# ucuapps/OpenGlue

Measured on AMD Instinct MI355X. Metric: image-pairs/sec (1024 kpts, 256-dim, 9 GNN layers), higher is better.
Workload: dtype f32; 1 GPU; BASELINE configs[1]: 1024x1024 kpts, 256-dim, 9 self+cross stages, 4 heads, 100 Sinkhorn iters, batch=32 pairs/GPU, random-init weights, seeded synthetic keypoints/descriptors; global_batch=32, pairs_per_gpu=32, parallelism=pairs sharded over 1 GPU(s), 1 RCCL gather

## Files before the change

openglue_amd/build.py:

```python
from __future__ import annotations

import argparse
import os
import shutil
import subprocess
import sys
from concurrent.futures import ThreadPoolExecutor

HERE = os.path.dirname(os.path.abspath(__file__))
CSRC = os.path.join(HERE, "csrc")
LIB_DIR = os.path.join(HERE, "lib")
LIB_PATH = os.path.join(LIB_DIR, "libopenglue_amd.so")
SOURCES = ["gemm_f32.hip", "gemm_f16x3.hip", "mlp_fused.hip", "attention.hip", "attention_train.hip", "linear_attention.hip", "sinkhorn.hip", "sinkhorn_resident.hip", "sinkhorn_train.hip", "batchnorm_train.hip", "matches.hip", "features.hip", "supervision.hip", "metrics.hip", "superpoint.hip", "optimizer.hip", "api.hip"]
ARCH = "gfx950"


def _hipcc() -> str:
    for cand in (os.environ.get("HIPCC"), shutil.which("hipcc"), "/opt/rocm/bin/hipcc"):
        if cand and os.path.exists(cand):
            return cand
    raise RuntimeError("hipcc not found (set HIPCC or install ROCm under /opt/rocm)")


_NO_PACKED_FP32 = ["-Xclang", "-target-feature", "-Xclang", "-packed-fp32-ops"]
PER_FILE_FLAGS = {"attention.hip": _NO_PACKED_FP32}
FLAGS = ["--offload-arch=" + ARCH, "-std=c++17", "-fPIC", "-O3", "-Wall", "-Wno-unused-function"]


def _stale(target: str, deps) -> bool:
    if not os.path.exists(target):
        return True
    t = os.path.getmtime(target)
    return any(os.path.getmtime(d) > t for d in deps)


def build(force: bool = False, debug: bool = False, verbose: bool = True) -> str:
    os.makedirs(LIB_DIR, exist_ok=True)
    hipcc = _hipcc()
    headers = [os.path.join(CSRC, "og_common.h"), os.path.join(os.path.dirname(HERE), "include", "openglue_amd.h")]
    flags = list(FLAGS)
    if debug:
        flags += ["-g", "-save-temps=obj"]
    objs, jobs = [], []
    for src in SOURCES:
        sp = os.path.join(CSRC, src)
        op = os.path.join(LIB_DIR, src.replace(".hip", ".o"))
        objs.append(op)
        if force or _stale(op, [sp, *headers, os.path.abspath(__file__)]):
            jobs.append([hipcc, *flags, *PER_FILE_FLAGS.get(src, []), "-c", sp, "-o", op])

    def run(cmd):
        if verbose:
            print(" ".join(cmd), flush=True)
        r = subprocess.run(cmd, capture_output=True, text=True)
        if r.returncode != 0:
            raise RuntimeError("hipcc failed:\n" + r.stdout + r.stderr)
        err = "\n".join(l for l in r.stderr.splitlines() if "is not a recognized feature for this target" not in l)
        if err.strip() and verbose:
            print(err, file=sys.stderr)

    with ThreadPoolExecutor(max_workers=max(1, min(len(jobs), os.cpu_count() or 1))) as ex:
        list(ex.map(run, jobs))
    if jobs or force or _stale(LIB_PATH, objs):
        run([hipcc, "--offload-arch=" + ARCH, "-shared", "-fPIC", "-o", LIB_PATH, *objs])
    return LIB_PATH


if __name__ == "__main__":
    ap = argparse.ArgumentParser()
    ap.add_argument("--force", action="store_true")
    ap.add_argument("--debug", action="store_true")
    a = ap.parse_args()
    print(build(force=a.force, debug=a.debug))
```

openglue_amd/csrc/api.hip:

```cpp
#include <math.h>
#include <cmath>
#include <stdlib.h>
#include <string.h>
#include <vector>
#include <dlfcn.h>
#include <stdio.h>

#include "og_common.h"

namespace {

constexpr double BN_EPS = 1e-5;

struct PackedLayout {
    int n_enc;
    int enc_k[OG_MAX_HIDDEN + 1];
    int enc_out[OG_MAX_HIDDEN + 1];
    int64_t enc_w[OG_MAX_HIDDEN + 1], enc_b[OG_MAX_HIDDEN + 1];
    int64_t enc_whl;
    int64_t layer0, layer_stride;
    int64_t o_wqkv, o_bqkv, o_w0, o_b0, o_w3, o_b3;
    int64_t o_wmlp;
    int64_t o_wqkvs;
    int64_t o_wqkvb;
// ... 363 lines not shown
            push = (int (*)(const char*))dlsym(h, "roctxRangePushA");
            pop = (int (*)())dlsym(h, "roctxRangePop");
            if (push && pop) return;
            push = nullptr; pop = nullptr;
        }
    }
};
struct Range {
    static const Roctx& rt() { static const Roctx r; return r; }
    bool on;
    explicit Range(const char* name) : on(rt().push != nullptr) { if (on) rt().push(name); }
    Range(const char* name, int idx) : on(rt().push != nullptr) {
        if (on) { char buf[48]; snprintf(buf, sizeof buf, "%s %d", name, idx); rt().push(buf); }
    }
    ~Range() { if (on) rt().pop(); }
    Range(const Range&) = delete;
};
struct Scope {
    Profiler* p; int i;
    Scope(Profiler* pp, int c) : p(pp), i(pp ? pp->begin(c) : -1) {}
    ~Scope() { if (p) p->end(i); }
};

int forward_impl(const og_shape* shape, const og_inputs* in, const void* packed_dev, void* workspace_dev,
                 const og_outputs* outp, void* stream, Profiler* prof, const RaggedDesc* rag = nullptr,
                 const EncoderRagged* er0 = nullptr, const EncoderRagged* er1 = nullptr, int tap = -1, float* tap_x = nullptr,
                 bool encoder_only = false) {
    static const og_outputs no_outputs{};
    if (encoder_only && !outp) outp = &no_outputs;
    if (!shape || !in || !packed_dev || !workspace_dev || !outp) return OG_E_INVALID;
    if (int e = check_shape(shape)) return e;
    og_clear_status();
    const og_shape& s = *shape;
    if (!in->keypoints0 || !in->keypoints1 || !in->descriptors0 || !in->descriptors1 || (!outp->scores && !encoder_only)) return OG_E_INVALID;
    if (s.side_info > 0 && (!in->side_info0 || !in->side_info1)) return OG_E_INVALID;
    if ((outp->matches0 == nullptr) != (outp->matching_scores0 == nullptr)) return OG_E_INVALID;
    if ((outp->matches1 == nullptr) != (outp->matching_scores1 == nullptr)) return OG_E_INVALID;
    if (outp->matches1 && !outp->matches0) return OG_E_INVALID;
    if (((uintptr_t)packed_dev & 15) || ((uintptr_t)workspace_dev & 15) || ((uintptr_t)in->descriptors0 & 15) ||
        ((uintptr_t)in->descriptors1 & 15))
        return OG_E_ALIGN;
    hipStream_t st = (hipStream_t)stream;
    const PackedLayout L = packed_layout(s);
    const WorkspaceLayout W = workspace_layout(s);
    const float* pk = (const float*)packed_dev;
    float* ws = (float*)workspace_dev;
    const int D = s.desc_dim, D2 = 2 * D, B = s.batch, m = s.m, n = s.n;
    const bool favor = s.flags & OG_FLAG_FAVOR_RELU;
    const int WQ = qk_width(s), QW = qkv_width(s);
    const int64_t T0 = rag ? rag->off0[B] : (int64_t)B * m, T1 = rag ? rag->off1[B] : (int64_t)B * n, T = T0 + T1;
    float* X32 = ws + W.x32; float* G = ws + W.g; float* Sb = ws + W.sbuf;
    const int D4 = 4 * D;
    _Float16* XO = (_Float16*)(ws + W.xo);
    _Float16* QKVh = (_Float16*)(ws + W.qkvh); _Float16* QKVl = (_Float16*)(ws + W.qkvl);
    _Float16* Hb = (_Float16*)(ws + W.h);
    int rc;

    auto gemm = [&](const float* A, int64_t lda, const float* Bm, int64_t ldb, float* C, int64_t ldc, int64_t M, int N, int K,
                    const float* bias, int relu, const float* res, int64_t ldr, _Float16* Chl, int64_t ldch) -> int {
        GemmArgs g{};
        g.A = A; g.lda = lda; g.strideA = 0; g.B = Bm; g.ldb = ldb; g.strideB = 0; g.C = C; g.ldc = ldc; g.strideC = 0;
        g.M = (int)M; g.N = N; g.K = K; g.batch = 1; g.bias = bias; g.relu = relu; g.res = res; g.ldr = ldr; g.strideR = 0;
        g.alpha = nullptr; g.scale = 1.f; g.Ct = nullptr; g.ldct = 0; g.strideCt = 0; g.ct_rows = 1;
        g.Ch = Chl; g.Cl = Chl ? Chl + 32 : nullptr; g.ldch = ldch; g.c_hl = 1;
        Scope sc(prof, OG_STAGE_GEMM);
        return og_launch_gemm(g, st);
    };
    auto gemmh = [&](const _Float16* A, const float* wbase, int64_t o_w, int64_t wrow0, int64_t M, int N, int K,
                     const float* bias, int relu, const _Float16* res_hl, float* C32, _Float16* Ch, _Float16* Cl, int64_t ldch,
                     int c_hl) -> int {
        GemmHArgs g{};
        g.scale_dev = wbase + L.o_scale + (o_w == L.o_wqkv ? 0 : o_w == L.o_w0 ? 1 : 2);
        g.A = A; g.lda = D4;
        g.B = (const _Float16*)(wbase + o_w) + wrow0 * 2 * K; g.ldb = 2 * K;
        g.M = (int)M; g.N = N; g.K = K; g.scale = (float)(1.0 / OG_W_SCALE); g.bias = bias; g.relu = relu; g.res = nullptr; g.ldr = D; g.res_hl = res_hl; g.ldrh = D4;
        g.C32 = C32; g.ldc = D; g.Ch = Ch; g.Cl = Cl; g.ldch = ldch; g.c_hl = c_hl;
        Scope sc(prof, OG_STAGE_GEMM_F16X3);
        return og_launch_gemm_f16x3(g, st);
    };

    Range r_forward("og_forward");
    {
        Range r_stage("encoder");
        float* EI = ws + W.ei;
        float* Ea = ws + W.ea;
        float* Eb = ws + W.eb;
        {
            Scope sc(prof, OG_STAGE_ENCODER_INPUT);
            if ((rc = og_launch_encoder_input(in->keypoints0, in->side_info0, T0, s.side_info, in->image0_wh[0], in->image0_wh[1], EI, st, er0))) return rc;
            if ((rc = og_launch_encoder_input(in->keypoints1, in->side_info1, T1, s.side_info, in->image1_wh[0], in->image1_wh[1], EI + T0 * 32, st, er1))) return rc;
        }
        const float* cur = EI; int64_t ldcur = 32;
        const bool tail_f16 = L.enc_whl >= 0;
        const int last = L.n_enc - 1;
        _Float16* Ehl = (_Float16*)G;
        for (int i = 0; i < L.n_enc; ++i) {
            const float* Wi = pk + L.enc_w[i]; const float* bi = pk + L.enc_b[i];
            if (i < last) {
                float* dst = (i & 1) ? Eb : Ea;
                const int act = (s.flags & OG_FLAG_SIREN_ENCODER) ? 2 : 1;
                const bool to_hl = tail_f16 && i == last - 1;
                if ((rc = gemm(cur, ldcur, Wi, L.enc_k[i], to_hl ? nullptr : dst, L.enc_maxw, T, L.enc_out[i], L.enc_k[i], bi, act, nullptr, 0,
                               to_hl ? Ehl : nullptr, to_hl ? 2 * L.enc_out[i] : 0))) return rc;
                cur = dst; ldcur = L.enc_maxw;
            } else {
                const bool nd = s.flags & OG_FLAG_NO_DESCRIPTORS;
                const float* res[2] = {nd ? nullptr : in->descriptors0, nd ? nullptr : in->descriptors1};
                const int64_t r0[2] = {0, T0}, R[2] = {T0, T1};
                for (int side = 0; side < 2; ++side) {
                    if (tail_f16) {
                        const int K = L.enc_k[i];
                        GemmHArgs g{};
                        g.A = Ehl + r0[side] * 2 * K; g.lda = 2 * K;
                        g.B = (const _Float16*)(pk + L.enc_whl); g.ldb = 2 * K;
                        g.M = (int)R[side]; g.N = D; g.K = K; g.scale = (float)(1.0 / OG_W_SCALE); g.scale_dev = pk + L.scales + 1; g.bias = bi; g.relu = 0;
                        g.res = res[side]; g.ldr = D; g.res_hl = nullptr; g.ldrh = 0;
                        g.C32 = nullptr; g.ldc = D; g.Ch = XO + r0[side] * D4; g.Cl = g.Ch + 32; g.ldch = D4; g.c_hl = 1;
                        Scope sc(prof, OG_STAGE_GEMM_F16X3);
                        if ((rc = og_launch_gemm_f16x3(g, st))) return rc;
                    } else {
                        if ((rc = gemm(cur + r0[side] * ldcur, ldcur, Wi, L.enc_k[i], X32 + r0[side] * D, D, R[side], D, L.enc_k[i], bi, 0, res[side], D,
                                       XO + r0[side] * D4, D4))) return rc;
                    }
                }
            }
        }
    }

    auto tap_here = [&](int idx) -> int {
        if (tap != idx || !tap_x) return 0;
        return og_launch_merge_f16_hl(XO, T, D, D4, tap_x, D, st);
    };
    if ((rc = tap_here(0))) return rc;
    if (encoder_only) return og_launch_status();

    const int dh = D / s.num_heads;
    if (hipMemsetAsync(ws + W.attn, 0, OG_ATTN_COUNTERS * sizeof(int), st) != hipSuccess) return OG_E_INVALID;
    auto attention = [&](int nz, int split, int64_t qb0, int64_t qs0, int nq0, int64_t kb0, int64_t ks0, int nk0,
                         int64_t qb1, int64_t qs1, int nq1, int64_t kb1, int64_t ks1, int nk1, int rag_mode) -> int {
        AttnArgs a{};
        a.rag = rag; a.rag_mode = rag_mode;
        a.qh = QKVh; a.ql = QKVl; a.ldq = QW; a.kh = QKVh + WQ; a.kl = QKVl + WQ; a.ldk = QW;
        a.vh = QKVh + 2 * WQ; a.vl = QKVl + 2 * WQ; a.ldv = QW;
        a.feat = favor ? WQ : 0;
        a.oh = XO + D2; a.ol = XO + D2 + 32; a.ldo = D4; a.o_hl = 1;
        a.nz = nz; a.num_heads = s.num_heads; a.dh = dh; a.split = split;
        a.counters = reinterpret_cast<int*>(ws + W.attn); a.partial = ws + W.attn + OG_ATTN_COUNTERS;
        a.q_base[0] = qb0; a.q_step[0] = qs0; a.nq[0] = nq0; a.kv_base[0] = kb0; a.kv_step[0] = ks0; a.nk[0] = nk0;
        a.q_base[1] = qb1; a.q_step[1] = qs1; a.nq[1] = nq1; a.kv_base[1] = kb1; a.kv_step[1] = ks1; a.nk[1] = nk1;
        Scope sc(prof, OG_STAGE_ATTENTION);
        if (favor) return og_launch_favor_attention(a, st);
        return (s.flags & OG_FLAG_LINEAR_ATTENTION) ? og_launch_linear_attention(a, st) : og_launch_attention(a, st);
    };
    auto proj_small_ok = [&](int64_t R) {
        static const int mode = [] { const char* e = getenv("OG_PROJ_SMALL"); return e ? atoi(e) : -1; }();
        return L.o_wqkvs >= 0 && !favor && (mode >= 0 ? mode != 0 : R <= 8192) && R < ((int64_t)1 << 30);
    };
    auto proj_small = [&](const float* lw, int64_t r0, int64_t R, int split_row, int a0, int a1, int b0, int b1) -> int {
        Scope sc(prof, OG_STAGE_GEMM_F16X3);
        return og_launch_proj_small(XO + r0 * D4, D4, (int)R, D, (const char*)(lw + L.o_wqkvs), lw + L.o_bqkv, lw + L.o_scale,
                                    QKVh + r0 * QW, QKVl + r0 * QW, QW, split_row, a0, a1, b0, b1, st);
    };
    auto proj_stream_ok = [&](int64_t R, bool full = false) {
        return L.o_wqkvb >= 0 && !favor && og_proj_stream_wanted((int)(R < ((int64_t)1 << 30) ? R : 0), D, full) && R < ((int64_t)1 << 30) && QW % 64 == 0 &&
               !(((uintptr_t)QKVh | (uintptr_t)QKVl) & 127);
    };
    auto proj_stream = [&](const float* lw, int64_t r0, int64_t R, int split_row, int a0, int a1, int b0, int b1) -> int {
        Scope sc(prof, OG_STAGE_GEMM_F16X3);
        return og_launch_proj_stream(XO + r0 * D4, D4, (int)R, D, (const char*)(lw + L.o_wqkvb), lw + L.o_bqkv, lw + L.o_scale,
                                     QKVh + r0 * QW, QKVl + r0 * QW, QW, split_row, a0 / 128, a1 / 128, b0 / 128, b1 / 128, st);
    };
    auto qkv_proj = [&](const float* lw, int64_t r0, int64_t R, int c0, int c1) -> int {
        if (proj_small_ok(R) && c0 % 32 == 0 && c1 % 32 == 0) return proj_small(lw, r0, R, 0, 0, 0, c0 / 32, c1 / 32);
        if (proj_stream_ok(R, c0 == 0 && c1 == QW) && c0 % 128 == 0 && c1 % 128 == 0 && ((r0 * QW * 2) % 128 == 0)) return proj_stream(lw, r0, R, 0, 0, 0, c0, c1);
        const int cut = favor ? 2 * WQ : c1;
        const int ca[2] = {c0, c0 < cut && cut < c1 ? cut : c1}, cb[2] = {ca[1], c1};
        for (int part = 0; part < 2; ++part) {
            const int a0 = part ? cb[0] : ca[0], a1 = part ? cb[1] : ca[1];
            if (a1 <= a0) continue;
// ... 213 lines not shown
```

openglue_amd/csrc/og_common.h:

```cpp
#pragma once
#include <hip/hip_runtime.h>
#include <stdint.h>
#include "../../include/openglue_amd.h"

typedef float f32x4 __attribute__((ext_vector_type(4)));
typedef float f32x16 __attribute__((ext_vector_type(16)));
typedef _Float16 f16x4 __attribute__((ext_vector_type(4)));
typedef _Float16 f16x8 __attribute__((ext_vector_type(8)));

#define OG_WAVE 64
#define OG_NEG_INF (-__builtin_huge_valf())

__device__ __forceinline__ int mfma32_row(int r, int lane) { return (r & 3) + 8 * (r >> 2) + 4 * (lane >> 5); }

__device__ __forceinline__ float wave_max(float v) {
#pragma unroll
    for (int o = 32; o > 0; o >>= 1) v = fmaxf(v, __shfl_xor(v, o, 64));
    return v;
}
__device__ __forceinline__ float wave_sum(float v) {
#pragma unroll
    for (int o = 32; o > 0; o >>= 1) v += __shfl_xor(v, o, 64);
    return v;
}
// ... 111 lines not shown
int og_launch_split_f16_hl(const float* x, int64_t rows, int cols, int64_t ldx, void* out, int64_t ldo, hipStream_t stream);
int og_launch_merge_f16_hl(const void* in, int64_t rows, int cols, int64_t ldi, float* out, int64_t ldo, hipStream_t stream);

struct MlpFusedArgs {
    _Float16* XO; int64_t ld;
    int M;
    const char* wstream;
    const float* b0;
    const float* b3;
    float scale;
    const float* scales_dev;
};
bool og_mlp_fused_supported(int D);
bool og_mlp_fused_enabled(int D);
size_t og_mlp_stream_bytes(int D);
bool og_pack_mlp_stream(int D, const double* W0, const double* W3, void* out, double S0 = OG_W_SCALE, double S3 = OG_W_SCALE);
int og_launch_mlp_fused(const MlpFusedArgs& a, int D, hipStream_t stream);
bool og_mlp_small_wanted(int M);
size_t og_proj_stream_bytes(int N, int K);
bool og_pack_proj_stream(int N, int K, const double* W, void* out, double S);
size_t og_proj_stream_big_bytes(int N, int K);
bool og_pack_proj_stream_big(int N, int K, const double* W, void* out, double S);
bool og_proj_stream_wanted(int M, int K, bool full);
int og_launch_proj_stream(const _Float16* X, int64_t ld, int M, int K, const char* wstream, const float* bias, const float* scale_dev,
                          _Float16* Ch, _Float16* Cl, int64_t ldc, int split_row, int a0, int a1, int b0, int b1, hipStream_t stream);
int og_launch_proj_small(const _Float16* X, int64_t ld, int M, int K, const char* wstream, const float* bias, const float* scale_dev,
                         _Float16* Ch, _Float16* Cl, int64_t ldc, int split_row, int a0, int a1, int b0, int b1, hipStream_t stream);

constexpr int OG_ATTN_COUNTERS = 256;
constexpr int64_t OG_ATTN_PARTIAL_FLOATS = (int64_t)512 * 4 * 34 * 64;
struct AttnArgs {
    const _Float16* qh; const _Float16* ql; int64_t ldq;
    const _Float16* kh; const _Float16* kl; int64_t ldk;
    const _Float16* vh; const _Float16* vl; int64_t ldv;
    _Float16* oh; _Float16* ol; int64_t ldo;
    int o_hl;
    int nz, num_heads, dh;
    int split;
    int64_t q_base[2], q_step[2], kv_base[2], kv_step[2];
    int nq[2], nk[2];
    int qtiles;
    const RaggedDesc* rag;
    int rag_mode;
    int feat;
    float* lse;
    float* partial;
    int* counters;
    int gs_scatter;
    int mx;
    int mx_scale_a;
    int mx_sv;
};
int og_launch_attention(const AttnArgs& a, hipStream_t stream);
int og_launch_linear_attention(const AttnArgs& a, hipStream_t stream);
int og_launch_favor_attention(const AttnArgs& a, hipStream_t stream);

struct RowBest { int* idx; float* val; int stride; };
int og_launch_sinkhorn(const float* S, int64_t lds, const float* dustbin_dev , float dustbin_host, int batch, int m, int n, int iters,
                       float reg, float* scores, void* workspace, hipStream_t stream, const RaggedDesc* rag = nullptr,
                       const RowBest* row_best = nullptr, bool trusted_padding = true);
bool og_sinkhorn_resident_shape_ok(int B, int m, int n);
size_t og_sinkhorn_resident_ws_bytes(int B, int m, int n);
bool og_sinkhorn_resident_wanted(int B, int m, int n, int mode);
int og_sinkhorn_resident_rounds(int B, int m, int n);
bool og_sinkhorn_resident_ragged_wanted(const RaggedDesc& rd, int mode);
int og_launch_sinkhorn_resident_ragged(const float* S, int64_t lds, const float* zdev, float zhost, const RaggedDesc& rd, int m_max, int n_max, int iters,
                                       float inv_reg, float* u, int ldu, const float* v_in, float* v_out, int ldv, void* xws, unsigned* status,
                                       hipStream_t st, bool trusted_padding = true, int* count_only = nullptr);
static inline bool og_sinkhorn_resident_ragged_wanted(const RaggedNone&, int) { return false; }
int og_launch_sinkhorn_resident(const float* S, int64_t lds, const float* zdev, float zhost, int B, int m, int n, int iters,
                                float inv_reg, float la, float la_bin, float lb, float lb_bin, float* u, int ldu, const float* v_in,
                                float* v_out, int ldv, void* xws, unsigned* status , hipStream_t st, bool trusted_padding = true);
int og_launch_matches(const float* scores, int batch, int m, int n, float thr, int64_t* matches0,
                      float* ms0, int64_t* matches1, float* ms1, void* workspace, hipStream_t stream,
                      const RaggedDesc* rag = nullptr, bool rows_done = false);
RowBest og_matches_row_best(void* matches_workspace, int batch, int m, int n);
struct EncoderRagged {
    int B;
    int off[OG_MAX_RAGGED + 1];
    float wm1[OG_MAX_RAGGED], hm1[OG_MAX_RAGGED];
};
int og_launch_encoder_input(const float* kpts, const float* side, int64_t tokens, int s, float wx, float wy,
                            float* out , hipStream_t stream, const EncoderRagged* er = nullptr);
```

Measured before the change: 3620 image-pairs/s.

## Fuse keypoint encoder input, hidden MLP layers and f16x3 tail into one kernel

Adds a single kernel that builds the normalized keypoint/side-info input, runs the hidden f32 MLP layers on MFMA, and computes the final split-f16 projection with the descriptor residual, writing the hi/lo output directly. Each wave keeps a 32-token tile in LDS, so intermediate activations never go to global memory and several launches collapse into one. The fused path is taken by default when shapes qualify and can be disabled with an environment variable. The cost is low occupancy (two waves per block) and duplicated encoder logic that must stay numerically consistent with the unfused path.

```diff
diff --git a/openglue_amd/build.py b/openglue_amd/build.py
--- a/openglue_amd/build.py
+++ b/openglue_amd/build.py
@@ -11,7 +11,7 @@
 CSRC = os.path.join(HERE, "csrc")
 LIB_DIR = os.path.join(HERE, "lib")
 LIB_PATH = os.path.join(LIB_DIR, "libopenglue_amd.so")
-SOURCES = ["gemm_f32.hip", "gemm_f16x3.hip", "mlp_fused.hip", "attention.hip", "attention_train.hip", "linear_attention.hip", "sinkhorn.hip", "sinkhorn_resident.hip", "sinkhorn_train.hip", "batchnorm_train.hip", "matches.hip", "features.hip", "supervision.hip", "metrics.hip", "superpoint.hip", "optimizer.hip", "api.hip"]
+SOURCES = ["gemm_f32.hip", "gemm_f16x3.hip", "mlp_fused.hip", "attention.hip", "attention_train.hip", "linear_attention.hip", "sinkhorn.hip", "sinkhorn_resident.hip", "sinkhorn_train.hip", "batchnorm_train.hip", "matches.hip", "features.hip", "encoder_fused.hip", "supervision.hip", "metrics.hip", "superpoint.hip", "optimizer.hip", "api.hip"]
 ARCH = "gfx950"
 
 
diff --git a/openglue_amd/csrc/api.hip b/openglue_amd/csrc/api.hip
--- a/openglue_amd/csrc/api.hip
+++ b/openglue_amd/csrc/api.hip
@@ -469,19 +469,38 @@
     Range r_forward("og_forward");
     {
         Range r_stage("encoder");
+        const bool tail_f16 = L.enc_whl >= 0;
+        static const bool fused_off = [] { const char* e = getenv("OG_ENCODER_FUSED"); return e && atoi(e) == 0; }();
+        bool fused = false;
+        if (tail_f16 && !fused_off && !rag && !er0 && !er1 && !(s.flags & OG_FLAG_SIREN_ENCODER)) {
+            EncoderFusedArgs a{};
+            a.kpts0 = in->keypoints0; a.kpts1 = in->keypoints1; a.side0 = in->side_info0; a.side1 = in->side_info1;
+            a.T0 = T0; a.T = T; a.s = s.side_info;
+            a.wm1[0] = in->image0_wh[0] - 1.f; a.hm1[0] = in->image0_wh[1] - 1.f; a.wm1[1] = in->image1_wh[0] - 1.f; a.hm1[1] = in->image1_wh[1] - 1.f;
+            a.n_hidden = L.n_enc - 1;
+            for (int i = 0; i < a.n_hidden && i < OG_MAX_HIDDEN; ++i) { a.W[i] = pk + L.enc_w[i]; a.b[i] = pk + L.enc_b[i]; a.K[i] = L.enc_k[i]; a.N[i] = L.enc_out[i]; }
+            a.Whl = (const _Float16*)(pk + L.enc_whl); a.bias_last = pk + L.enc_b[L.n_enc - 1]; a.scale_dev = pk + L.scales + 1;
+            const bool nd = s.flags & OG_FLAG_NO_DESCRIPTORS;
+            a.res0 = nd ? nullptr : in->descriptors0; a.res1 = nd ? nullptr : in->descriptors1;
+            a.XO = XO; a.ldxo = D4;
+            if (og_encoder_fused_supported(a, D)) {
+                Scope sc(prof, OG_STAGE_GEMM);
+                if ((rc = og_launch_encoder_fused(a, D, st))) return rc;
+                fused = true;
+            }
+        }
         float* EI = ws + W.ei;
         float* Ea = ws + W.ea;
         float* Eb = ws + W.eb;
-        {
+        if (!fused) {
             Scope sc(prof, OG_STAGE_ENCODER_INPUT);
             if ((rc = og_launch_encoder_input(in->keypoints0, in->side_info0, T0, s.side_info, in->image0_wh[0], in->image0_wh[1], EI, st, er0))) return rc;
             if ((rc = og_launch_encoder_input(in->keypoints1, in->side_info1, T1, s.side_info, in->image1_wh[0], in->image1_wh[1], EI + T0 * 32, st, er1))) return rc;
         }
         const float* cur = EI; int64_t ldcur = 32;
-        const bool tail_f16 = L.enc_whl >= 0;
         const int last = L.n_enc - 1;
         _Float16* Ehl = (_Float16*)G;
-        for (int i = 0; i < L.n_enc; ++i) {
+        for (int i = 0; i < L.n_enc && !fused; ++i) {
             const float* Wi = pk + L.enc_w[i]; const float* bi = pk + L.enc_b[i];
             if (i < last) {
                 float* dst = (i & 1) ? Eb : Ea;
diff --git a/openglue_amd/csrc/encoder_fused.hip b/openglue_amd/csrc/encoder_fused.hip
--- /dev/null
+++ b/openglue_amd/csrc/encoder_fused.hip
@@ -0,0 +1,241 @@
+#include "og_common.h"
+
+namespace {
+
+constexpr int EF_WAVES = 2;
+constexpr int EF_LDH = 2 * 64 + 8;
+constexpr int EF_SLAB_ROWB = 128 + 16;
+
+template <int K>
+__device__ __forceinline__ void ef_conv_f32_k(const float* act, int lda, const float* __restrict__ W, int c0, f32x16 (&acc)[2], int lane) {
+    const int l31 = lane & 31, hi = lane >> 5;
+    const float* ap = act + l31 * lda + 4 * hi;
+    const float* wp = W + (int64_t)(c0 + l31) * K + 4 * hi;
+    f32x4 a[K / 8], b[K / 8][2];
+#pragma unroll
+    for (int kk = 0; kk < K / 8; ++kk) {
+#pragma unroll
+        for (int t = 0; t < 2; ++t) b[kk][t] = *reinterpret_cast<const f32x4*>(wp + t * 32 * K + 8 * kk);
+    }
+#pragma unroll
+    for (int kk = 0; kk < K / 8; ++kk) a[kk] = *reinterpret_cast<const f32x4*>(ap + 8 * kk);
+#pragma unroll
+    for (int t = 0; t < 2; ++t)
+#pragma unroll
+        for (int r = 0; r < 16; ++r) acc[t][r] = 0.f;
+#pragma unroll
+    for (int kk = 0; kk < K / 8; ++kk)
+#pragma unroll
+        for (int e = 0; e < 4; ++e)
+#pragma unroll
+            for (int t = 0; t < 2; ++t) acc[t] = __builtin_amdgcn_mfma_f32_32x32x2f32(a[kk][e], b[kk][t][e], acc[t], 0, 0, 0);
+}
+__device__ __forceinline__ void ef_conv_f32(const float* act, int lda, const float* __restrict__ W, int K, int c0, f32x16 (&acc)[2], int lane) {
+    if (K == 32) ef_conv_f32_k<32>(act, lda, W, c0, acc, lane);
+    else if (K == 64) ef_conv_f32_k<64>(act, lda, W, c0, acc, lane);
+    else ef_conv_f32_k<128>(act, lda, W, c0, acc, lane);
+}
+
+template <int D>
+__global__ __launch_bounds__(64 * EF_WAVES) void encoder_fused_kernel(EncoderFusedArgs g) {
+    constexpr int TI = D / 32;
+    extern __shared__ __attribute__((aligned(16))) char ef_smem[];
+    const int lane = threadIdx.x & 63;
+    const int wave = __builtin_amdgcn_readfirstlane(threadIdx.x >> 6);
+    const int l31 = lane & 31, hi = lane >> 5;
+    const int64_t tok0 = ((int64_t)blockIdx.x * EF_WAVES + wave) * 32;
+    if (tok0 >= g.T) return;
+    char* base = ef_smem + (size_t)wave * g.wave_bytes;
+    float* cur = reinterpret_cast<float*>(base);
+    float* nxt = reinterpret_cast<float*>(base + g.off_q);
+    _Float16* H = reinterpret_cast<_Float16*>(base + g.off_h);
+    const int ldp = g.ldp;
+
+#pragma unroll
+    for (int it = 0; it < 4; ++it) {
+        const int r = it * 8 + (lane >> 3), c4 = (lane & 7) * 4;
+        const int64_t t = tok0 + r;
+        f32x4 o = {0.f, 0.f, 0.f, 0.f};
+        if (t < g.T) {
+            const int im = t >= g.T0;
+            const int64_t tt = im ? t - g.T0 : t;
+            const float* kp = im ? g.kpts1 : g.kpts0;
+            const float* sd = im ? g.side1 : g.side0;
+            const float wm1 = g.wm1[im], hm1 = g.hm1[im];
+#pragma unroll
+            for (int e = 0; e < 4; ++e) {
+                const int c = c4 + e;
+                float v = 0.f;
+                if (c == 0) v = 2.f * kp[2 * tt] / wm1 - 1.f;
+                else if (c == 1) v = 2.f * kp[2 * tt + 1] / hm1 - 1.f;
+                else if (c < 2 + g.s) v = sd[tt * g.s + (c - 2)];
+                o[e] = v;
+            }
+        }
+        *reinterpret_cast<f32x4*>(cur + r * ldp + c4) = o;
+    }
+    __builtin_amdgcn_wave_barrier();
+
+    f32x16 acc[2];
+    for (int i = 0; i + 1 < g.n_hidden; ++i) {
+#pragma clang fp contract(off)
+        const int K = g.K[i], N = g.N[i];
+        for (int c0 = 0; c0 < N; c0 += 64) {
+            ef_conv_f32(cur, ldp, g.W[i], K, c0, acc, lane);
+#pragma unroll
+            for (int t = 0; t < 2; ++t) {
+                const int col = c0 + 32 * t + l31;
+                const float bias = g.b[i][col];
+#pragma unroll
+                for (int r = 0; r < 16; ++r) {
+                    float v = acc[t][r] + bias;
+                    v = fmaxf(v, 0.f);
+                    nxt[mfma32_row(r, lane) * ldp + col] = v;
+                }
+            }
+        }
+        __builtin_amdgcn_wave_barrier();
+        float* sw = cur; cur = nxt; nxt = sw;
+    }
+
+    const int il = g.n_hidden - 1;
+    const int KL = g.N[il];
+    const float scale = *g.scale_dev, inv_scale = 1.f / scale;
+    f32x16 xa[TI];
+#pragma unroll
+    for (int i = 0; i < TI; ++i)
+#pragma unroll
+        for (int q = 0; q < 4; ++q) {
+            const f32x4 b = *reinterpret_cast<const f32x4*>(g.bias_last + i * 32 + 8 * q + 4 * hi) * inv_scale;
+#pragma unroll
+            for (int e = 0; e < 4; ++e) xa[i][4 * q + e] = b[e];
+        }
+    const _Float16* wl_row = g.Whl + (int64_t)l31 * 2 * KL + hi * 8;
+    f16x8 wh[2][TI], wl[2][TI];
+    auto load_w = [&](int kt, int ks, f16x8 (&h)[TI], f16x8 (&l)[TI]) {
+#pragma unroll
+        for (int i = 0; i < TI; ++i) {
+            const _Float16* wp = wl_row + (int64_t)i * 32 * 2 * KL + kt * 64 + 16 * ks;
+            h[i] = *reinterpret_cast<const f16x8*>(wp);
+            l[i] = *reinterpret_cast<const f16x8*>(wp + 32);
+        }
+    };
+    const int64_t tok = tok0 + l31;
+    const int64_t tokc = tok < g.T ? tok : g.T - 1;
+    const float* rp = nullptr;
+    if (g.res0) rp = (tokc >= g.T0 ? g.res1 + (tokc - g.T0) * D : g.res0 + tokc * D) + 4 * hi;
+    f32x4 rr[4][4];
+    auto load_res = [&](int i, f32x4 (&d)[4]) {
+#pragma unroll
+        for (int q = 0; q < 4; ++q) d[q] = *reinterpret_cast<const f32x4*>(rp + i * 32 + 8 * q);
+    };
+    if (rp) {
+#pragma unroll
+        for (int i = 0; i < 4; ++i) load_res(i, rr[i]);
+    }
+    for (int c0 = 0; c0 < KL; c0 += 64) {
+        load_w(c0 / 32, 0, wh[0], wl[0]);
+        {
+#pragma clang fp contract(off)
+            ef_conv_f32(cur, ldp, g.W[il], g.K[il], c0, acc, lane);
+#pragma unroll
+            for (int t = 0; t < 2; ++t) {
+                const float bias = g.b[il][c0 + 32 * t + l31];
+#pragma unroll
+                for (int r = 0; r < 16; ++r) {
+                    float v = acc[t][r] + bias;
+                    v = fmaxf(v, 0.f);
+                    _Float16* d = H + mfma32_row(r, lane) * EF_LDH + 64 * t + l31;
+                    og_split(v, d[0], d[32]);
+                }
+            }
+        }
+        __builtin_amdgcn_wave_barrier();
+#pragma unroll
+        for (int st = 0; st < 4; ++st) {
+            const int t = st >> 1, ks = st & 1;
+            if (st + 1 < 4) load_w(c0 / 32 + ((st + 1) >> 1), (st + 1) & 1, wh[(st + 1) & 1], wl[(st + 1) & 1]);
+            const f16x8 xh = *reinterpret_cast<const f16x8*>(H + l31 * EF_LDH + 64 * t + 16 * ks + 8 * hi);
+            const f16x8 xl = *reinterpret_cast<const f16x8*>(H + l31 * EF_LDH + 64 * t + 16 * ks + 8 * hi + 32);
+#pragma unroll
+            for (int i = 0; i < TI; ++i) xa[i] = __builtin_amdgcn_mfma_f32_32x32x16_f16(wl[st & 1][i], xh, xa[i], 0, 0, 0);
+#pragma unroll
+            for (int i = 0; i < TI; ++i) xa[i] = __builtin_amdgcn_mfma_f32_32x32x16_f16(wh[st & 1][i], xl, xa[i], 0, 0, 0);
+#pragma unroll
+            for (int i = 0; i < TI; ++i) xa[i] = __builtin_amdgcn_mfma_f32_32x32x16_f16(wh[st & 1][i], xh, xa[i], 0, 0, 0);
+        }
+        __builtin_amdgcn_wave_barrier();
+    }
+
+    {
+#pragma clang fp contract(off)
+        char* slab = reinterpret_cast<char*>(cur);
+#pragma unroll
+        for (int i = 0; i < TI; ++i) {
+#pragma unroll
+            for (int r = 0; r < 16; ++r) xa[i][r] = fmaxf(xa[i][r] * scale, OG_NEG_INF);
+            if (rp) {
+#pragma unroll
+                for (int q = 0; q < 4; ++q)
+#pragma unroll
+                    for (int e = 0; e < 4; ++e) xa[i][4 * q + e] += rr[i & 3][q][e];
+                if (i + 4 < TI) load_res(i + 4, rr[i & 3]);
+            }
+#pragma unroll
+            for (int q = 0; q < 4; ++q) {
+                unsigned ha, la, hb, lb;
+                og_split4(xa[i][4 * q], xa[i][4 * q + 1], xa[i][4 * q + 2], xa[i][4 * q + 3], ha, la, hb, lb);
+                char* d = slab + l31 * EF_SLAB_ROWB + (8 * q + 4 * hi) * 2;
+                *reinterpret_cast<uint2*>(d) = make_uint2(ha, hb);
+                *reinterpret_cast<uint2*>(d + 64) = make_uint2(la, lb);
+            }
+            __builtin_amdgcn_wave_barrier();
+#pragma unroll
+            for (int it = 0; it < 4; ++it) {
+                const int r = it * 8 + (lane >> 3), c = lane & 7;
+                const f16x8 t = *reinterpret_cast<const f16x8*>(slab + r * EF_SLAB_ROWB + c * 16);
+                const int64_t tk = tok0 + r;
+                if (tk < g.T) *reinterpret_cast<f16x8*>(g.XO + tk * g.ldxo + og_hl_col(i * 32) + c * 8) = t;
+            }
+            __builtin_amdgcn_wave_barrier();
+        }
+    }
+}
+
+}
+
+bool og_encoder_fused_supported(const EncoderFusedArgs& a, int D) {
+    if (D != 128 && D != 256) return false;
+    if (a.n_hidden < 1 || a.n_hidden > OG_MAX_HIDDEN || a.K[0] != 32) return false;
+    for (int i = 0; i < a.n_hidden; ++i) {
+        if (a.N[i] <= 0 || a.N[i] > 128 || a.N[i] % 64 || (a.K[i] != 32 && a.K[i] != 64 && a.K[i] != 128)) return false;
+        if (i > 0 && a.K[i] != a.N[i - 1]) return false;
+    }
+    return a.T > 0 && a.T < ((int64_t)1 << 36);
+}
+
+int og_launch_encoder_fused(const EncoderFusedArgs& args, int D, hipStream_t st) {
+    EncoderFusedArgs a = args;
+    if (!og_encoder_fused_supported(a, D)) return OG_E_SHAPE;
+    if (!a.kpts0 || !a.kpts1 || !a.XO || !a.Whl || !a.bias_last || !a.scale_dev || (a.s > 0 && (!a.side0 || !a.side1)) || a.s < 0 || 2 + a.s > 32 ||
+        (a.res0 == nullptr) != (a.res1 == nullptr))
+        return OG_E_INVALID;
+    int maxw = 32;
+    for (int i = 0; i + 1 < a.n_hidden; ++i) maxw = a.N[i] > maxw ? a.N[i] : maxw;
+    a.ldp = maxw + 4;
+    const int pbytes = 32 * a.ldp * (int)sizeof(float);
+    a.off_q = pbytes;
+    a.off_h = a.n_hidden > 1 ? 2 * pbytes : pbytes;
+    a.wave_bytes = a.off_h + 32 * EF_LDH * (int)sizeof(_Float16);
+    const size_t shmem = (size_t)EF_WAVES * a.wave_bytes;
+    const int64_t groups = (a.T + 31) / 32;
+    const unsigned grid = (unsigned)((groups + EF_WAVES - 1) / EF_WAVES);
+    if (shmem > 65536) {
+        const hipError_t e = D == 256 ? hipFuncSetAttribute((const void*)encoder_fused_kernel<256>, hipFuncAttributeMaxDynamicSharedMemorySize, (int)shmem)
+                                      : hipFuncSetAttribute((const void*)encoder_fused_kernel<128>, hipFuncAttributeMaxDynamicSharedMemorySize, (int)shmem);
+        if (e != hipSuccess) return (int)e;
+    }
+    if (D == 256) hipLaunchKernelGGL(encoder_fused_kernel<256>, dim3(grid), dim3(64 * EF_WAVES), shmem, st, a);
+    else hipLaunchKernelGGL(encoder_fused_kernel<128>, dim3(grid), dim3(64 * EF_WAVES), shmem, st, a);
+    return og_launch_status();
+}
diff --git a/openglue_amd/csrc/og_common.h b/openglue_amd/csrc/og_common.h
--- a/openglue_amd/csrc/og_common.h
+++ b/openglue_amd/csrc/og_common.h
@@ -217,3 +217,21 @@
 };
 int og_launch_encoder_input(const float* kpts, const float* side, int64_t tokens, int s, float wx, float wy,
                             float* out , hipStream_t stream, const EncoderRagged* er = nullptr);
+struct EncoderFusedArgs {
+    const float* kpts0; const float* kpts1;
+    const float* side0; const float* side1;
+    int64_t T0, T;
+    int s;
+    float wm1[2], hm1[2];
+    int n_hidden;
+    const float* W[OG_MAX_HIDDEN]; const float* b[OG_MAX_HIDDEN];
+    int K[OG_MAX_HIDDEN], N[OG_MAX_HIDDEN];
+    const _Float16* Whl;
+    const float* bias_last;
+    const float* scale_dev;
+    const float* res0; const float* res1;
+    _Float16* XO; int64_t ldxo;
+    int ldp, off_q, off_h, wave_bytes;
+};
+bool og_encoder_fused_supported(const EncoderFusedArgs& a, int D);
+int og_launch_encoder_fused(const EncoderFusedArgs& a, int D, hipStream_t stream);
```

After: 3622 image-pairs/s, median of 2. No clear change (+0.0%).

## Fuse keypoint encoder MLP into a single LDS-resident kernel

Applied to the files above, without the earlier changes.

Adds one kernel that runs the whole keypoint encoder for a 128-token tile: input normalisation, three fp32 MFMA layers with activations kept in LDS, and the final f16x3 split-precision projection with descriptor residual add. It writes the hi/lo f16 layout straight into the transformer input buffer. This replaces two encoder-input launches plus four GEMM launches and their global-memory round trips for intermediate activations. It is on by default when the layer shapes match, and can be switched off with an environment variable. The encoder is a small part of a 9-layer GNN plus 100 Sinkhorn iterations, so the overall gain is limited.

```diff
diff --git a/openglue_amd/build.py b/openglue_amd/build.py
--- a/openglue_amd/build.py
+++ b/openglue_amd/build.py
@@ -11,7 +11,7 @@
 CSRC = os.path.join(HERE, "csrc")
 LIB_DIR = os.path.join(HERE, "lib")
 LIB_PATH = os.path.join(LIB_DIR, "libopenglue_amd.so")
-SOURCES = ["gemm_f32.hip", "gemm_f16x3.hip", "mlp_fused.hip", "attention.hip", "attention_train.hip", "linear_attention.hip", "sinkhorn.hip", "sinkhorn_resident.hip", "sinkhorn_train.hip", "batchnorm_train.hip", "matches.hip", "features.hip", "supervision.hip", "metrics.hip", "superpoint.hip", "optimizer.hip", "api.hip"]
+SOURCES = ["gemm_f32.hip", "gemm_f16x3.hip", "mlp_fused.hip", "attention.hip", "attention_train.hip", "linear_attention.hip", "sinkhorn.hip", "sinkhorn_resident.hip", "sinkhorn_train.hip", "batchnorm_train.hip", "matches.hip", "features.hip", "encoder.hip", "supervision.hip", "metrics.hip", "superpoint.hip", "optimizer.hip", "api.hip"]
 ARCH = "gfx950"
 
 
diff --git a/openglue_amd/csrc/api.hip b/openglue_amd/csrc/api.hip
--- a/openglue_amd/csrc/api.hip
+++ b/openglue_amd/csrc/api.hip
@@ -469,10 +469,25 @@
     Range r_forward("og_forward");
     {
         Range r_stage("encoder");
+        const bool enc_fused = og_encoder_fused_enabled() && L.enc_whl >= 0 && T <= 0x7fffffff &&
+                               og_encoder_fused_supported(L.n_enc, L.enc_k, L.enc_out, D, s.side_info);
+        if (enc_fused) {
+            const bool nd = s.flags & OG_FLAG_NO_DESCRIPTORS;
+            EncFusedArgs e{};
+            e.kpts[0] = in->keypoints0; e.kpts[1] = in->keypoints1; e.side[0] = in->side_info0; e.side[1] = in->side_info1;
+            e.desc[0] = nd ? nullptr : in->descriptors0; e.desc[1] = nd ? nullptr : in->descriptors1;
+            e.wm1[0] = in->image0_wh[0] - 1.f; e.hm1[0] = in->image0_wh[1] - 1.f; e.wm1[1] = in->image1_wh[0] - 1.f; e.hm1[1] = in->image1_wh[1] - 1.f;
+            e.T0 = (int)T0; e.T = (int)T; e.s = s.side_info; e.D = D; e.act = (s.flags & OG_FLAG_SIREN_ENCODER) ? 2 : 1;
+            e.w0 = pk + L.enc_w[0]; e.b0 = pk + L.enc_b[0]; e.w1 = pk + L.enc_w[1]; e.b1 = pk + L.enc_b[1]; e.w2 = pk + L.enc_w[2]; e.b2 = pk + L.enc_b[2];
+            e.whl = (const _Float16*)(pk + L.enc_whl); e.b3 = pk + L.enc_b[3]; e.scale_dev = pk + L.scales + 1;
+            e.XO = XO; e.ldx = D4;
+            Scope sc(prof, OG_STAGE_GEMM);
+            if ((rc = og_launch_encoder_fused(e, er0, er1, st))) return rc;
+        }
         float* EI = ws + W.ei;
         float* Ea = ws + W.ea;
         float* Eb = ws + W.eb;
-        {
+        if (!enc_fused) {
             Scope sc(prof, OG_STAGE_ENCODER_INPUT);
             if ((rc = og_launch_encoder_input(in->keypoints0, in->side_info0, T0, s.side_info, in->image0_wh[0], in->image0_wh[1], EI, st, er0))) return rc;
             if ((rc = og_launch_encoder_input(in->keypoints1, in->side_info1, T1, s.side_info, in->image1_wh[0], in->image1_wh[1], EI + T0 * 32, st, er1))) return rc;
@@ -481,7 +496,7 @@
         const bool tail_f16 = L.enc_whl >= 0;
         const int last = L.n_enc - 1;
         _Float16* Ehl = (_Float16*)G;
-        for (int i = 0; i < L.n_enc; ++i) {
+        for (int i = 0; i < L.n_enc && !enc_fused; ++i) {
             const float* Wi = pk + L.enc_w[i]; const float* bi = pk + L.enc_b[i];
             if (i < last) {
                 float* dst = (i & 1) ? Eb : Ea;
diff --git a/openglue_amd/csrc/encoder.hip b/openglue_amd/csrc/encoder.hip
--- /dev/null
+++ b/openglue_amd/csrc/encoder.hip
@@ -0,0 +1,297 @@
+#include <stdlib.h>
+#include <type_traits>
+
+#include "og_common.h"
+
+namespace {
+
+constexpr int ET = 128;
+constexpr int ENT = 512;
+constexpr int LD0 = 32 + 4;
+constexpr int LD1 = 64 + 4;
+constexpr int SLAB = 32 * 144;
+constexpr int P_BYTES = ET * 512;
+constexpr int Q_BYTES = 8 * SLAB;
+static_assert(ET * LD1 * 4 <= P_BYTES && ET * LD1 * 4 <= Q_BYTES && ET * LD0 * 4 <= Q_BYTES, "activation tiles must fit their regions");
+
+struct EncRagged2 { EncoderRagged e[2]; };
+struct EncRaggedNone {};
+
+__device__ __forceinline__ int enc_pair_of(const EncoderRagged& er, int t) {
+    int lo = 0, hi = er.B - 1;
+    while (lo < hi) {
+        const int mid = (lo + hi + 1) >> 1;
+        if (er.off[mid] <= t) lo = mid; else hi = mid - 1;
+    }
+    return lo;
+}
+
+template <int K, int TN>
+__device__ __forceinline__ void enc_load_w(const float* __restrict__ W, int col0, int lane, f32x4 (&bw)[K / 8][TN]) {
+#pragma unroll
+    for (int kk = 0; kk < K / 8; ++kk)
+#pragma unroll
+        for (int j = 0; j < TN; ++j)
+            bw[kk][j] = *reinterpret_cast<const f32x4*>(W + (int64_t)(col0 + j * 32 + (lane & 31)) * K + kk * 8 + (lane >> 5) * 4);
+}
+
+template <int K, int TN, int LDA>
+__device__ __forceinline__ void enc_mma(const float* As, int rb, int lane, const f32x4 (&bw)[K / 8][TN], f32x16 (&acc)[TN]) {
+#pragma unroll
+    for (int j = 0; j < TN; ++j)
+#pragma unroll
+        for (int r = 0; r < 16; ++r) acc[j][r] = 0.f;
+    const float* ap = As + (rb * 32 + (lane & 31)) * LDA + (lane >> 5) * 4;
+#pragma unroll
+    for (int kk = 0; kk < K / 8; ++kk) {
+        const f32x4 a = *reinterpret_cast<const f32x4*>(ap + kk * 8);
+#pragma unroll
+        for (int e = 0; e < 4; ++e)
+#pragma unroll
+            for (int j = 0; j < TN; ++j) acc[j] = __builtin_amdgcn_mfma_f32_32x32x2f32(a[e], bw[kk][j][e], acc[j], 0, 0, 0);
+    }
+}
+
+__device__ __forceinline__ float enc_act(float v, int act) {
+    if (act == 1) v = fmaxf(v, 0.f);
+    else if (act == 2) v = sinf(30.f * v);
+    return v;
+}
+
+template <class ER>
+__global__ __launch_bounds__(ENT) void encoder_fused_kernel(EncFusedArgs g, ER er) {
+    __shared__ __attribute__((aligned(128))) char smem[P_BYTES + Q_BYTES];
+    char* const Pb = smem;
+    char* const Qb = smem + P_BYTES;
+    float* const Pf = reinterpret_cast<float*>(Pb);
+    float* const Qf = reinterpret_cast<float*>(Qb);
+
+    const int tid = threadIdx.x, lane = tid & 63;
+    const int wave = __builtin_amdgcn_readfirstlane(tid >> 6);
+    const int rb = wave >> 1, ch = wave & 1;
+    const int l31 = lane & 31, hi = lane >> 5;
+    const int row0 = blockIdx.x * ET;
+
+    f32x4 bw0[4][1];
+    enc_load_w<32, 1>(g.w0, ch * 32, lane, bw0);
+
+    {
+        const int r = tid >> 2, c8 = (tid & 3) * 8;
+        const int grow = row0 + r;
+        f32x4 o[2] = {f32x4{0.f, 0.f, 0.f, 0.f}, f32x4{0.f, 0.f, 0.f, 0.f}};
+        if (grow < g.T) {
+            const int im = grow >= g.T0 ? 1 : 0;
+            const int64_t t = grow - (im ? g.T0 : 0);
+            const float* __restrict__ kpts = g.kpts[im];
+            const float* __restrict__ side = g.side[im];
+            float wm1 = g.wm1[im], hm1 = g.hm1[im];
+            if constexpr (!std::is_same<ER, EncRaggedNone>::value) {
+                const int b = enc_pair_of(er.e[im], (int)t);
+                wm1 = er.e[im].wm1[b]; hm1 = er.e[im].hm1[b];
+            }
+            const int s = g.s;
+#pragma unroll
+            for (int e = 0; e < 8; ++e) {
+                const int c = c8 + e;
+                float v = 0.f;
+                if (c == 0) v = 2.f * kpts[2 * t] / wm1 - 1.f;
+                else if (c == 1) v = 2.f * kpts[2 * t + 1] / hm1 - 1.f;
+                else if (c < 2 + s) v = side[t * s + (c - 2)];
+                o[e >> 2][e & 3] = v;
+            }
+        }
+        *reinterpret_cast<f32x4*>(Qf + r * LD0 + c8) = o[0];
+        *reinterpret_cast<f32x4*>(Qf + r * LD0 + c8 + 4) = o[1];
+    }
+    __syncthreads();
+
+    f32x4 bw1[8][1];
+    {
+        f32x16 acc[1];
+        enc_mma<32, 1, LD0>(Qf, rb, lane, bw0, acc);
+        enc_load_w<64, 1>(g.w1, ch * 32, lane, bw1);
+        {
+#pragma clang fp contract(off)
+            const int col = ch * 32 + l31;
+            const float bias = g.b0[col];
+#pragma unroll
+            for (int r = 0; r < 16; ++r) {
+                const float v = enc_act(acc[0][r] + bias, g.act);
+                Pf[(rb * 32 + mfma32_row(r, lane)) * LD1 + col] = v;
+            }
+        }
+    }
+    __syncthreads();
+
+    f32x4 bw2[8][2];
+    {
+        f32x16 acc[1];
+        enc_mma<64, 1, LD1>(Pf, rb, lane, bw1, acc);
+        enc_load_w<64, 2>(g.w2, ch * 64, lane, bw2);
+        {
+#pragma clang fp contract(off)
+            const int col = ch * 32 + l31;
+            const float bias = g.b1[col];
+#pragma unroll
+            for (int r = 0; r < 16; ++r) {
+                const float v = enc_act(acc[0][r] + bias, g.act);
+                Qf[(rb * 32 + mfma32_row(r, lane)) * LD1 + col] = v;
+            }
+        }
+    }
+    __syncthreads();
+
+    const int ngrp = g.D >> 5;
+    const int oc0 = (wave & (ngrp - 1)) * 32;
+    const int tb0 = wave / ngrp, tbs = 8 / ngrp;
+    const int swz = (l31 >> 1) & 7;
+    char* const slab = Qb + wave * SLAB;
+    f16x8 wh[4][2], wl[4][2];
+    {
+        const _Float16* wp = g.whl + (int64_t)(oc0 + l31) * 256 + hi * 8;
+#pragma unroll
+        for (int kt = 0; kt < 4; ++kt)
+#pragma unroll
+            for (int ks = 0; ks < 2; ++ks) {
+                wh[kt][ks] = *reinterpret_cast<const f16x8*>(wp + kt * 64 + ks * 16);
+                wl[kt][ks] = *reinterpret_cast<const f16x8*>(wp + kt * 64 + ks * 16 + 32);
+            }
+    }
+    f32x4 bias4[4];
+#pragma unroll
+    for (int q = 0; q < 4; ++q) bias4[q] = *reinterpret_cast<const f32x4*>(g.b3 + oc0 + 8 * q + 4 * hi);
+    const float scale = *g.scale_dev;
+    const float inv_scale = 1.f / scale;
+    f32x4 dl[4];
+    auto load_desc = [&](int tokb) {
+        if (!g.desc[0]) return;
+#pragma unroll
+        for (int it = 0; it < 4; ++it) {
+            int tk = tokb + it * 8 + (lane >> 3);
+            tk = tk < g.T ? tk : g.T - 1;
+            const float* dp = tk >= g.T0 ? g.desc[1] + (int64_t)(tk - g.T0) * g.D : g.desc[0] + (int64_t)tk * g.D;
+            dl[it] = *reinterpret_cast<const f32x4*>(dp + oc0 + (lane & 7) * 4);
+        }
+    };
+#pragma unroll
+    for (int it = 0; it < 4; ++it) dl[it] = f32x4{0.f, 0.f, 0.f, 0.f};
+    load_desc(row0 + tb0 * 32);
+
+
+    {
+        f32x16 acc[2];
+        enc_mma<64, 2, LD1>(Qf, rb, lane, bw2, acc);
+        {
+#pragma clang fp contract(off)
+#pragma unroll
+            for (int j = 0; j < 2; ++j) {
+                const int col = ch * 64 + j * 32 + l31;
+                const float bias = g.b2[col];
+                char* const slabp = Pb + (col >> 5) * (ET * 128);
+                const int c = (col & 31) >> 3;
+#pragma unroll
+                for (int r = 0; r < 16; ++r) {
+                    const int row = rb * 32 + mfma32_row(r, lane);
+                    const float v = enc_act(acc[j][r] + bias, g.act);
+                    _Float16 h, l;
+                    og_split(v, h, l);
+                    const int off = row * 128 + ((c ^ ((row >> 1) & 7)) * 16) + (col & 7) * 2;
+                    *reinterpret_cast<_Float16*>(slabp + off) = h;
+                    *reinterpret_cast<_Float16*>(slabp + (off ^ 64)) = l;
+                }
+            }
+        }
+    }
+    __syncthreads();
+
+    for (int tb = tb0; tb < ET / 32; tb += tbs) {
+        const int tokb = row0 + tb * 32;
+        f32x4 dcur[4];
+#pragma unroll
+        for (int it = 0; it < 4; ++it) dcur[it] = dl[it];
+        if (tb + tbs < ET / 32) load_desc(tokb + tbs * 32);
+        f32x16 acc;
+#pragma unroll
+        for (int q = 0; q < 4; ++q) {
+            const f32x4 b = bias4[q] * inv_scale;
+#pragma unroll
+            for (int e = 0; e < 4; ++e) acc[4 * q + e] = b[e];
+        }
+        const int x_row = (tb * 32 + l31) * 128;
+#pragma unroll
+        for (int kt = 0; kt < 4; ++kt) {
+            const char* sb = Pb + kt * (ET * 128);
+#pragma unroll
+            for (int ks = 0; ks < 2; ++ks) {
+                const int cho = ((2 * ks + hi) ^ swz) * 16;
+                const f16x8 xh = *reinterpret_cast<const f16x8*>(sb + x_row + cho);
+                const f16x8 xl = *reinterpret_cast<const f16x8*>(sb + x_row + (cho ^ 64));
+                acc = __builtin_amdgcn_mfma_f32_32x32x16_f16(wl[kt][ks], xh, acc, 0, 0, 0);
+                acc = __builtin_amdgcn_mfma_f32_32x32x16_f16(wh[kt][ks], xl, acc, 0, 0, 0);
+                acc = __builtin_amdgcn_mfma_f32_32x32x16_f16(wh[kt][ks], xh, acc, 0, 0, 0);
+            }
+        }
+        {
+#pragma clang fp contract(off)
+#pragma unroll
+            for (int r = 0; r < 16; ++r) acc[r] = acc[r] * scale;
+            if (g.desc[0]) {
+#pragma unroll
+                for (int it = 0; it < 4; ++it) *reinterpret_cast<f32x4*>(slab + (it * 8 + (lane >> 3)) * 144 + (lane & 7) * 16) = dcur[it];
+#pragma unroll
+                for (int q = 0; q < 4; ++q) {
+                    const f32x4 rr = *reinterpret_cast<const f32x4*>(slab + l31 * 144 + (8 * q + 4 * hi) * 4);
+#pragma unroll
+                    for (int e = 0; e < 4; ++e) acc[4 * q + e] += rr[e];
+                }
+            }
+#pragma unroll
+            for (int q = 0; q < 4; ++q) {
+                unsigned ha, la, hb, lb;
+                og_split4(acc[4 * q], acc[4 * q + 1], acc[4 * q + 2], acc[4 * q + 3], ha, la, hb, lb);
+                char* d = slab + l31 * 144 + (8 * q + 4 * hi) * 2;
+                *reinterpret_cast<uint2*>(d) = make_uint2(ha, hb);
+                *reinterpret_cast<uint2*>(d + 64) = make_uint2(la, lb);
+            }
+#pragma unroll
+            for (int it = 0; it < 4; ++it) {
+                const int r = it * 8 + (lane >> 3), c = lane & 7;
+                const f16x8 t = *reinterpret_cast<const f16x8*>(slab + r * 144 + c * 16);
+                const int tk = tokb + r;
+                if (tk < g.T) *reinterpret_cast<f16x8*>(g.XO + (int64_t)tk * g.ldx + og_hl_col(oc0) + c * 8) = t;
+            }
+        }
+    }
+}
+
+}
+
+bool og_encoder_fused_enabled() {
+    static const bool on = [] { const char* e = getenv("OG_ENCODER_FUSED"); return !e || atoi(e) != 0; }();
+    return on;
+}
+
+bool og_encoder_fused_supported(int n_enc, const int* enc_k, const int* enc_out, int D, int side_info) {
+    if (n_enc != 4 || (D != 128 && D != 256) || side_info < 0 || 2 + side_info > 32) return false;
+    return enc_k[0] == 32 && enc_out[0] == 64 && enc_k[1] == 64 && enc_out[1] == 64 && enc_k[2] == 64 && enc_out[2] == 128 &&
+           enc_k[3] == 128 && enc_out[3] == D;
+}
+
+int og_launch_encoder_fused(const EncFusedArgs& a, const EncoderRagged* er0, const EncoderRagged* er1, hipStream_t stream) {
+    if (!a.kpts[0] || !a.kpts[1] || !a.XO || !a.w0 || !a.b0 || !a.w1 || !a.b1 || !a.w2 || !a.b2 || !a.whl || !a.b3 || !a.scale_dev) return OG_E_INVALID;
+    if (a.T <= 0 || a.T0 < 0 || a.T0 > a.T || (a.D != 128 && a.D != 256) || a.s < 0 || 2 + a.s > 32) return OG_E_INVALID;
+    if (a.s > 0 && (!a.side[0] || !a.side[1])) return OG_E_INVALID;
+    if ((a.desc[0] == nullptr) != (a.desc[1] == nullptr) || (er0 == nullptr) != (er1 == nullptr)) return OG_E_INVALID;
+    if (((uintptr_t)a.XO & 15) || (a.ldx & 7) || a.ldx < 2 * (int64_t)a.D || ((uintptr_t)a.desc[0] & 15) || ((uintptr_t)a.desc[1] & 15) ||
+        ((uintptr_t)a.w0 & 15) || ((uintptr_t)a.w1 & 15) || ((uintptr_t)a.w2 & 15) || ((uintptr_t)a.whl & 15) || ((uintptr_t)a.b3 & 15))
+        return OG_E_ALIGN;
+    const dim3 grid((unsigned)((a.T + ET - 1) / ET)), block(ENT);
+    if (er0) {
+        EncRagged2 e;
+        e.e[0] = *er0; e.e[1] = *er1;
+        hipLaunchKernelGGL(encoder_fused_kernel<EncRagged2>, grid, block, 0, stream, a, e);
+    } else {
+        hipLaunchKernelGGL(encoder_fused_kernel<EncRaggedNone>, grid, block, 0, stream, a, EncRaggedNone{});
+    }
+    return og_launch_status();
+}
diff --git a/openglue_amd/csrc/og_common.h b/openglue_amd/csrc/og_common.h
--- a/openglue_amd/csrc/og_common.h
+++ b/openglue_amd/csrc/og_common.h
@@ -217,3 +217,20 @@
 };
 int og_launch_encoder_input(const float* kpts, const float* side, int64_t tokens, int s, float wx, float wy,
                             float* out , hipStream_t stream, const EncoderRagged* er = nullptr);
+
+struct EncFusedArgs {
+    const float* kpts[2]; const float* side[2];
+    const float* desc[2];
+    float wm1[2], hm1[2];
+    int T0, T;
+    int s, D, act;
+    const float* w0; const float* b0;
+    const float* w1; const float* b1;
+    const float* w2; const float* b2;
+    const _Float16* whl; const float* b3;
+    const float* scale_dev;
+    _Float16* XO; int64_t ldx;
+};
+bool og_encoder_fused_enabled();
+bool og_encoder_fused_supported(int n_enc, const int* enc_k, const int* enc_out, int D, int side_info);
+int og_launch_encoder_fused(const EncFusedArgs& a, const EncoderRagged* er0, const EncoderRagged* er1, hipStream_t stream);
```

Result: no change. 3570 image-pairs/s before, 3590 image-pairs/s after, median of 6 (+0.6%).
